# ethz-asl/okvis

Hardware: NVIDIA B200
Metric: keyframe-window optimize() iters/sec (10KF/2k-lm stereo) (higher is better)
Workload: dtype f64

## Files before the change

okvis_b200/csrc/okb_estimator.cu:

```cuda
#include <cuda_runtime.h>

#include <algorithm>
#include <cstddef>
#include <cstdio>
#include <cstdlib>
#include <cstring>
#include <string>
#include <thread>
#include <vector>

#include "okb_ctx.h"
#include "okb_hostpack.hpp"
#include "okb_graph.cuh"
#include "okb_kernels.cuh"
#include "okb_marg.cuh"

using namespace okb;

static std::string g_create_error;

#define OKB_CUDA(ctx, call)                                                                             \
  do {                                                                                                  \
    cudaError_t e_ = (call);                                                                            \
    if (e_ != cudaSuccess) {                                                                            \
      (ctx)->set_error(std::string(#call) + ": " + cudaGetErrorString(e_));                             \
      return OKB_ERR_CUDA;                                                                              \
    }                                                                                                   \
  } while (0)

static inline size_t align_up(size_t v, size_t a) { return (v + a - 1) / a * a; }

static cudaError_t create_transfer_stream(cudaStream_t* s) {
  int lo = 0, hi = 0;
  cudaDeviceGetStreamPriorityRange(&lo, &hi);
  return cudaStreamCreateWithPriority(s, cudaStreamNonBlocking, hi);
}

extern "C" int okb_ctx_create(int device_id, int max_windows, okb_ctx** out) {
  if (!out || max_windows < 1) return OKB_ERR_INVALID_ARG;
  *out = nullptr;
  int n = 0;
  cudaError_t e = cudaGetDeviceCount(&n);
  if (e != cudaSuccess || n == 0) {
    g_create_error = std::string("no CUDA device: ") + cudaGetErrorString(e);
    return OKB_ERR_NO_DEVICE;
  }
  if (device_id < 0 || device_id >= n) { g_create_error = "bad device id"; return OKB_ERR_INVALID_ARG; }
  okb_ctx* c = new okb_ctx();
  c->device = device_id;
  c->max_windows = max_windows;
  int prio_least = 0, prio_greatest = 0;
  if (cudaSetDevice(device_id) == cudaSuccess) cudaDeviceGetStreamPriorityRange(&prio_least, &prio_greatest);
  if (cudaSetDevice(device_id) != cudaSuccess || cudaStreamCreateWithPriority(&c->stream, cudaStreamNonBlocking, prio_greatest) != cudaSuccess) {
    g_create_error = "cudaSetDevice / cudaStreamCreate failed";
    delete c;
    return OKB_ERR_CUDA;
  }
  if (cudaStreamCreateWithPriority(&c->stream_imu, cudaStreamNonBlocking, prio_least) != cudaSuccess ||
      cudaEventCreateWithFlags(&c->ev_round, cudaEventDisableTiming) != cudaSuccess ||
      cudaEventCreateWithFlags(&c->ev_imu, cudaEventDisableTiming) != cudaSuccess ||
      create_transfer_stream(&c->stream_xfer) != cudaSuccess ||
      cudaEventCreateWithFlags(&c->ev_join, cudaEventDisableTiming) != cudaSuccess) {
    g_create_error = "cudaStreamCreate / cudaEventCreate failed";
    delete c;
    return OKB_ERR_CUDA;
  }
  for (int k = 0; k < okb_ctx::kDoneRing; ++k) cudaEventCreateWithFlags(&c->done_ring[k], cudaEventDisableTiming);
  cudaDeviceProp prop;
  cudaGetDeviceProperties(&prop, device_id);
  c->sm_count = prop.multiProcessorCount;
  c->smem_optin = (int)prop.sharedMemPerBlockOptin;
  c->smem_per_sm = (int)prop.sharedMemPerMultiprocessor;
  c->wins.resize(max_windows);
  c->host.assign(max_windows, WinDev());
  std::memset(c->host.data(), 0, sizeof(WinDev) * max_windows);
  c->chunk_cap = std::max(1, std::min(kMaxChunks, (2 * c->sm_count) / max_windows));
  if (cudaMalloc(&c->d_wins, sizeof(WinDev) * max_windows) != cudaSuccess ||
      cudaMalloc(&c->d_states, sizeof(SolverState) * max_windows) != cudaSuccess ||
      cudaMallocHost(&c->h_states, sizeof(SolverState) * max_windows) != cudaSuccess) {
    g_create_error = "cudaMalloc failed";
    delete c;
    return OKB_ERR_CUDA;
  }
  cudaMemset(c->d_states, 0, sizeof(SolverState) * max_windows);
  cudaFuncSetAttribute(k_schur, cudaFuncAttributeMaxDynamicSharedMemorySize, c->smem_optin);
  cudaFuncSetAttribute(k_imu, cudaFuncAttributeMaxDynamicSharedMemorySize, (int)smemI_bytes());
  cudaFuncSetAttribute(k_imu, cudaFuncAttributePreferredSharedMemoryCarveout, cudaSharedmemCarveoutMaxShared);
  cudaFuncSetAttribute(k_solve<S_THREADS>, cudaFuncAttributeMaxDynamicSharedMemorySize, c->smem_optin);
  cudaFuncSetAttribute(k_solve<S_THREADS>, cudaFuncAttributePreferredSharedMemoryCarveout, cudaSharedmemCarveoutMaxShared);
  cudaFuncSetAttribute(k_solve<512>, cudaFuncAttributeMaxDynamicSharedMemorySize, c->smem_optin);
  cudaFuncSetAttribute(k_solve<512>, cudaFuncAttributePreferredSharedMemoryCarveout, cudaSharedmemCarveoutMaxShared);
  cudaFuncSetAttribute(k_schur, cudaFuncAttributePreferredSharedMemoryCarveout, cudaSharedmemCarveoutMaxShared);
  cudaFuncSetAttribute(k_quality, cudaFuncAttributeMaxDynamicSharedMemorySize, c->smem_optin);
  *out = c;
  return OKB_OK;
}

extern "C" void okb_ctx_destroy(okb_ctx* c) {
  if (!c) return;
  cudaSetDevice(c->device);
  cudaStreamSynchronize(c->stream);
  if (c->stream_xfer) cudaStreamSynchronize(c->stream_xfer);
  for (auto& w : c->wins) {
    if (w.arena) cudaFree(w.arena);
    if (w.marg_scratch) cudaFree(w.marg_scratch);
    if (w.staging) cudaFreeHost(w.staging);
    if (w.out_staging) cudaFreeHost(w.out_staging);
    if (w.copied) cudaEventDestroy(w.copied);
    if (w.down) cudaEventDestroy(w.down);
  }
  for (int k = 0; k < okb_ctx::kDoneRing; ++k) if (c->done_ring[k]) cudaEventDestroy(c->done_ring[k]);
  if (c->ev_join) cudaEventDestroy(c->ev_join);
  if (c->stream_xfer) cudaStreamDestroy(c->stream_xfer);
  okb_frontend_release(c);
  for (int r = 0; r < kMaxShard; ++r)
    if (c->shard_peer_ipc[r] && c->shard_peer[r]) cudaIpcCloseMemHandle(c->shard_peer[r]);
  if (c->shard_local) cudaFree(c->shard_local);
  if (c->d_wins) cudaFree(c->d_wins);
  if (c->d_states) cudaFree(c->d_states);
  if (c->h_states) cudaFreeHost(c->h_states);
  if (c->hook_buf) cudaFree(c->hook_buf);
  for (auto& g : c->graphs) if (g.exec) cudaGraphExecDestroy(g.exec);
  for (auto e : c->prof_events) cudaEventDestroy(e);
  if (c->ev_round) cudaEventDestroy(c->ev_round);
  if (c->ev_imu) cudaEventDestroy(c->ev_imu);
  if (c->stream_imu) cudaStreamDestroy(c->stream_imu);
  cudaStreamDestroy(c->stream);
  delete c;
}

extern "C" const char* okb_last_error(const okb_ctx* c) { return c ? c->error.c_str() : g_create_error.c_str(); }
extern "C" int64_t okb_kernel_launches(const okb_ctx* c) { return c ? c->launches : 0; }
extern "C" void* okb_stream(const okb_ctx* c) { return c ? (void*)c->stream : nullptr; }

namespace {
struct ArenaPlan {
  size_t total = 0;
  size_t take(size_t bytes) {
    const size_t o = total;
    total = align_up(total + bytes, 256);
    return o;
  }
};

int join_transfers(okb_ctx* c) {
  if (cudaEventRecord(c->ev_join, c->stream_xfer) != cudaSuccess) return 1;
  return cudaStreamWaitEvent(c->stream, c->ev_join, 0) != cudaSuccess;
}
void mark_work(okb_ctx* c, int first, int count) {
  const int k = c->done_next;
  c->done_next = (k + 1) % okb_ctx::kDoneRing;
  cudaEventRecord(c->done_ring[k], c->stream);
  for (int i = first; i < first + count; ++i) c->wins[i].done_idx = k;
}

inline bool caps_cover(const WinCaps& a, const WinCaps& b) {
  return a.K >= b.K && a.L >= b.L && a.O >= b.O && a.S >= b.S && a.T >= b.T && a.NE >= b.NE && a.NC >= b.NC && a.PP >= b.PP && a.MN >= b.MN;
}
inline WinCaps caps_max(const WinCaps& a, const WinCaps& b) {
  return WinCaps{std::max(a.K, b.K), std::max(a.L, b.L), std::max(a.O, b.O), std::max(a.S, b.S), std::max(a.T, b.T),
                 std::max(a.NE, b.NE), std::max(a.NC, b.NC), std::max(a.PP, b.PP), std::max(a.MN, b.MN)};
}
inline size_t full_upload_bytes(const WinCaps& q) {
  return 12 * sizeof(CmdHeader) + 8 * ((size_t)7 * q.NE + 16 * (size_t)q.K + 4 * (size_t)q.L + 2 * kMaxMargBlocks + 16 * kMaxMargBlocks +
                                        (size_t)q.MN * q.MN + q.MN) +
         sizeof(okb_camera) * q.NC + sizeof(okb_observation) * (size_t)q.O + sizeof(okb_imu_term) * q.T + sizeof(okb_imu_sample) * (size_t)q.S +
         (sizeof(okb_pose_prior) + sizeof(okb_sb_prior)) * q.PP + 4096;
}

void derive_dims(WinDev& W) {
  int CP = 1;
  while (CP < W.NC) CP <<= 1;
  W.CP = CP;
  W.NS = W.K * CP; W.NG = (W.NS + 31) / 32; W.NSP = W.NG * 32;
  W.dc = 6 * W.K; W.d = W.dc + 9 * W.NSB; W.dcp = 4 * ((W.dc + 1 + 3) / 4);
  W.Lp = (W.L + 31) & ~31;
// ... 780 lines not shown
  out[0] = (double)s.shard_rounds; out[1] = 1e-3 * (double)s.shard_wait_ns; out[2] = (double)s.shard_fault; out[3] = (double)s.shard_epoch;
  return OKB_OK;
}

static void prof_begin(okb_ctx* c, int kind) {
  if (!c->profile) return;
  if (c->prof_used + 2 > c->prof_events.size()) {
    cudaEvent_t a, b;
    cudaEventCreate(&a); cudaEventCreate(&b);
    c->prof_events.push_back(a); c->prof_events.push_back(b);
  }
  c->prof_kind.push_back(kind);
  cudaEventRecord(c->prof_events[c->prof_used], c->stream);
}
static void prof_end(okb_ctx* c) {
  if (!c->profile) return;
  cudaEventRecord(c->prof_events[c->prof_used + 1], c->stream);
  c->prof_used += 2;
}
extern "C" int okb_profile_enable(okb_ctx* c, int on) {
  if (!c) return OKB_ERR_INVALID_ARG;
  cudaSetDevice(c->device);
  cudaStreamSynchronize(c->stream);
  c->profile = on != 0;
  c->prof_used = 0;
  c->prof_kind.clear();
  return OKB_OK;
}
extern "C" int okb_profile_read(okb_ctx* c, double out[6]) {
  if (!c || !out) return OKB_ERR_INVALID_ARG;
  cudaSetDevice(c->device);
  cudaStreamSynchronize(c->stream);
  for (int i = 0; i < 6; ++i) out[i] = 0.0;
  for (size_t i = 0; i < c->prof_kind.size(); ++i) {
    float ms = 0.f;
    cudaEventElapsedTime(&ms, c->prof_events[2 * i], c->prof_events[2 * i + 1]);
    out[2 * c->prof_kind[i]] += ms;
    out[2 * c->prof_kind[i] + 1] += 1.0;
  }
  c->prof_used = 0;
  c->prof_kind.clear();
  return OKB_OK;
}

static int check_range(okb_ctx* c, int first, int count) {
  if (!c || first < 0 || count < 1 || first + count > c->max_windows) return OKB_ERR_INVALID_ARG;
  for (int i = first; i < first + count; ++i)
    if (!c->wins[i].uploaded) { c->set_error("window slot not uploaded"); return OKB_ERR_INVALID_ARG; }
  return OKB_OK;
}

extern "C" int64_t okb_window_h2d_bytes(const okb_ctx* c, int win) {
  if (!c || win < 0 || win >= c->max_windows || !c->wins[win].uploaded) return 0;
  return (int64_t)(c->wins[win].h2d_bytes + sizeof(WinDev));
}

extern "C" int okb_window_reset(okb_ctx* c, int first, int count) {
  int rc = check_range(c, first, count);
  if (rc) return rc;
  cudaSetDevice(c->device);
  for (int i = first; i < first + count; ++i) {
    const WinStore& S = c->wins[i];
    const WinDev& W = c->host[i];
    if (W.K != S.K_init || W.NSB != S.NSB_init || W.L != S.L_init) { c->set_error("okb_window_reset: the window changed shape since its last full upload"); return OKB_ERR_INVALID_ARG; }
  }
  rc = commit_range(c, first, count);
  if (rc) return rc;
  cudaStream_t xs = c->stream_xfer;
  bool waited[okb_ctx::kDoneRing] = {};
  for (int i = first; i < first + count; ++i) {
    const WinStore& S = c->wins[i];
    if (S.done_idx >= 0 && !waited[S.done_idx]) {
      OKB_CUDA(c, cudaStreamWaitEvent(xs, c->done_ring[S.done_idx], 0));
      waited[S.done_idx] = true;
    }
  }
  k_reset<<<count, 128, 0, xs>>>(c->d_wins, first, 1);
  c->launches += 1;
  OKB_CUDA(c, cudaGetLastError());
  return OKB_OK;
}

struct RoundPlan {
  int max_chunks = 1, max_imu = 0, max_cx = 1, max_K = 1, acc_copies = 1, chol_smem = 1, solve_threads = S_THREADS, gxQ = 1, shard = 0, push_gx = 1;
  size_t smA = 0, smS = 0, smQ = 0;
};
static int plan_rounds(okb_ctx* c, int first, int count, RoundPlan& P) {
  P = RoundPlan();
  int chol_smem = 1;
  int acc_copies = 1;
  const size_t sm_two = ((size_t)c->smem_per_sm - 2048) / 2;
  for (int i = first; i < first + count; ++i)
    if (smemA2_bytes(c->host[i].K, c->host[i].dcp, 1) > std::min((size_t)c->smem_optin, sm_two) &&
        smemA2_bytes(c->host[i].K, c->host[i].dcp, 0) <= sm_two) acc_copies = 0;
  for (int i = first; i < first + count; ++i)
    if (smemA2_bytes(c->host[i].K, c->host[i].dcp, acc_copies) > (size_t)c->smem_optin) acc_copies = 0;
  int maxL = 1;
  for (int i = first; i < first + count; ++i) {
    const WinDev& W = c->host[i];
    P.max_chunks = std::max(P.max_chunks, W.n_chunks);
    P.max_imu = std::max(P.max_imu, W.n_imu);
    P.smA = std::max(P.smA, smemA2_bytes(W.K, W.dcp, acc_copies));
    P.max_cx = std::max(P.max_cx, (W.L + L1_THREADS - 1) / L1_THREADS);
    P.max_K = std::max(P.max_K, W.K);
    {
      const int wm = smemS_bytes(W.d, W.dc, W.K, W.marg_n, W.n_imu, 1) <= (size_t)c->smem_optin ? 1
                   : smemS_bytes(W.d, W.dc, W.K, W.marg_n, W.n_imu, 2) <= (size_t)c->smem_optin ? 2 : 0;
      if (wm == 0 || chol_smem == 0) chol_smem = 0;
      else if (wm == 2) chol_smem = 2;
    }
    P.smQ = std::max(P.smQ, (size_t)W.NS * sizeof(SlotCtx));
    maxL = std::max(maxL, W.L);
  }
  for (int i = first; i < first + count; ++i) {
    const WinDev& W = c->host[i];
    P.smS = std::max(P.smS, smemS_bytes(W.d, W.dc, W.K, W.marg_n, W.n_imu, chol_smem));
  }
  if (P.smS > (size_t)c->smem_optin) { c->set_error("window does not fit kernel S shared memory"); return OKB_ERR_CAPACITY; }
  if (const char* force = getenv("OKB_SOLVE_MODE")) {
    const int m = atoi(force);
    if ((m == 0 || m == 2) && chol_smem != 0 && !(chol_smem == 2 && m == 2)) {
      chol_smem = m;
      P.smS = 0;
      for (int i = first; i < first + count; ++i) {
        const WinDev& W = c->host[i];
        P.smS = std::max(P.smS, smemS_bytes(W.d, W.dc, W.K, W.marg_n, W.n_imu, chol_smem));
      }
      if (P.smS > (size_t)c->smem_optin) { c->set_error("window does not fit kernel S shared memory"); return OKB_ERR_CAPACITY; }
    }
  }
  P.acc_copies = acc_copies; P.chol_smem = chol_smem;
  P.solve_threads = (2 * count <= c->sm_count) ? 512 : S_THREADS;
  P.gxQ = std::max(1, std::min((maxL + 127) / 128, (4 * c->sm_count + count - 1) / count));
  P.shard = c->shard_world > 1 ? 1 : 0;
  P.push_gx = std::max(1, std::min(16, c->sm_count / std::max(1, count)));
  return OKB_OK;
}

static int launch_rounds(okb_ctx* c, int first, int count, const okb_solve_options& opt, int rounds, const RoundPlan& P) {
  for (int r = 0; r < rounds; ++r) {
    const dim3 gridA(P.max_chunks, count);
    static const bool imu_serial = getenv("OKB_IMU_SERIAL") != nullptr;
    if (P.max_imu > 0 && imu_serial) {
      k_imu<<<dim3((P.max_imu + 32 / IMU_G - 1) / (32 / IMU_G), count), 32, smemI_bytes(), c->stream>>>(c->d_wins, first);
      c->launches += 1;
    } else if (P.max_imu > 0) {
      cudaEventRecord(c->ev_round, c->stream);
      cudaStreamWaitEvent(c->stream_imu, c->ev_round, 0);
      k_imu<<<dim3((P.max_imu + 32 / IMU_G - 1) / (32 / IMU_G), count), 32, smemI_bytes(), c->stream_imu>>>(c->d_wins, first);
      cudaEventRecord(c->ev_imu, c->stream_imu);
      c->launches += 1;
    }
    prof_begin(c, 0);
    k_linearize<<<dim3(P.max_cx, P.max_K, count), L1_THREADS, 0, c->stream>>>(c->d_wins, first);
    k_lmblock<<<dim3(P.max_cx, count), 128, 0, c->stream>>>(c->d_wins, first);
    k_schur<<<gridA, A2_THREADS, P.smA, c->stream>>>(c->d_wins, first, P.acc_copies, opt.max_iterations);
    if (P.shard) {
      k_shard_push<<<dim3(P.push_gx, count), 256, 0, c->stream>>>(c->d_wins, first);
      c->launches += 1;
    } else if (P.max_chunks > 1) { k_reduce_partials<<<dim3(8, count), 256, 0, c->stream>>>(c->d_wins, first); c->launches += 1; }
    prof_end(c);
    c->launches += 3;
    if (P.max_imu > 0 && !imu_serial) cudaStreamWaitEvent(c->stream, c->ev_imu, 0);
    prof_begin(c, 1);
    if (P.solve_threads == 512) k_solve<512><<<count, 512, P.smS, c->stream>>>(c->d_wins, first, opt, P.chol_smem);
    else k_solve<S_THREADS><<<count, S_THREADS, P.smS, c->stream>>>(c->d_wins, first, opt, P.chol_smem);
    prof_end(c);
    c->launches += 1;
  }
  OKB_CUDA(c, cudaGetLastError());
  return OKB_OK;
}

static int launch_quality(okb_ctx* c, int first, int count, const RoundPlan& P) {
  prof_begin(c, 2);
  k_quality<<<dim3(P.gxQ, count), 128, P.smQ, c->stream>>>(c->d_wins, first);
  prof_end(c);
  c->launches += 1;
  OKB_CUDA(c, cudaGetLastError());
  return OKB_OK;
}

static int run_rounds(okb_ctx* c, int first, int count, const okb_solve_options& opt, int rounds, bool with_quality) {
  RoundPlan P;
  int rc = plan_rounds(c, first, count, P);
  if (rc) return rc;
  static const bool no_graph = getenv("OKB_NO_GRAPH") != nullptr;
  if (c->profile || no_graph || c->shard_world > 1) {
    rc = launch_rounds(c, first, count, opt, rounds, P);
    if (!rc && with_quality) rc = launch_quality(c, first, count, P);
    return rc;
  }
  okb_ctx::GraphEntry key;
  std::memset(&key, 0, sizeof key);
  key.first = first; key.count = count; key.rounds = rounds; key.with_quality = with_quality ? 1 : 0;
  key.opt_iter = opt.max_iterations; key.opt_min = opt.min_iterations; key.opt_cauchy = opt.use_cauchy_loss; key.opt_time = opt.time_limit_s;
  static_assert(sizeof(RoundPlan) <= sizeof(key.plan), "plan blob");
  std::memcpy(key.plan, &P, sizeof P);
  for (auto& e : c->graphs)
    if (e.exec && !std::memcmp(&e, &key, offsetof(okb_ctx::GraphEntry, exec))) {
      e.stamp = ++c->graph_clock;
      OKB_CUDA(c, cudaGraphLaunch(e.exec, c->stream));
      c->launches += e.launches;
      return OKB_OK;
    }
  const int64_t l0 = c->launches;
  cudaGraph_t graph = nullptr;
  OKB_CUDA(c, cudaStreamBeginCapture(c->stream, cudaStreamCaptureModeThreadLocal));
  rc = launch_rounds(c, first, count, opt, rounds, P);
  if (!rc && with_quality) rc = launch_quality(c, first, count, P);
  const cudaError_t ce = cudaStreamEndCapture(c->stream, &graph);
  if (rc) { if (graph) cudaGraphDestroy(graph); return rc; }
  OKB_CUDA(c, ce);
  key.launches = c->launches - l0;
  c->launches = l0;
  OKB_CUDA(c, cudaGraphInstantiate(&key.exec, graph, 0));
  cudaGraphDestroy(graph);
  okb_ctx::GraphEntry* slot = nullptr;
  for (auto& e : c->graphs) if (!e.exec) { slot = &e; break; }
  if (!slot && c->graphs.size() < 16) { c->graphs.emplace_back(); slot = &c->graphs.back(); }
  if (!slot) {
    slot = &c->graphs[0];
    for (auto& e : c->graphs) if (e.stamp < slot->stamp) slot = &e;
    cudaGraphExecDestroy(slot->exec);
  }
  key.stamp = ++c->graph_clock;
  *slot = key;
  OKB_CUDA(c, cudaGraphLaunch(slot->exec, c->stream));
  c->launches += slot->launches;
  return OKB_OK;
}

extern "C" int okb_optimize_async(okb_ctx* c, int first, int count, const okb_solve_options* opt) {
  int rc = check_range(c, first, count);
  if (rc) return rc;
  if (!opt || opt->max_iterations < 0) return OKB_ERR_INVALID_ARG;
  cudaSetDevice(c->device);
  rc = commit_range(c, first, count);
  if (rc) return rc;
  for (int i = first; i < first + count; ++i) {
    WinDev& W = c->host[i];
    int chunks = (2 * c->sm_count + count - 1) / count;
    chunks = std::max(1, std::min(chunks, c->chunk_cap));
    chunks = std::min(chunks, std::max(1, W.L / (2 * A2_TILE)));
    W.lm_per_chunk = (((W.L + chunks - 1) / chunks) + A2_TILE - 1) / A2_TILE * A2_TILE;
    W.n_chunks = (W.L + W.lm_per_chunk - 1) / W.lm_per_chunk;
    W.use_cauchy = opt->use_cauchy_loss ? 1 : 0;
  }
  if (join_transfers(c)) { c->set_error("stream ordering failed"); return OKB_ERR_CUDA; }
  OKB_CUDA(c, cudaMemcpyAsync(c->d_wins + first, &c->host[first], sizeof(WinDev) * count, cudaMemcpyHostToDevice, c->stream));
  k_reset<<<count, 128, 0, c->stream>>>(c->d_wins, first, 0);
  c->launches += 1;
  for (int i = first; i < first + count; ++i) c->wins[i].opt = *opt;
  rc = run_rounds(c, first, count, *opt, opt->max_iterations + 1, true);
  if (rc) return rc;
  OKB_CUDA(c, cudaMemcpyAsync(c->h_states + first, c->d_states + first, sizeof(SolverState) * count, cudaMemcpyDeviceToHost, c->stream));
  mark_work(c, first, count);
  return rc;
}
// ... 418 lines not shown
```

okvis_b200/csrc/okb_kernels_lm.cuh:

```cuda
#pragma once
#include "okb_estimator.cuh"

namespace okb {

constexpr int L1_THREADS = 128;
constexpr int A2_THREADS = 192;
constexpr int A2_TILE = 32;
constexpr int kPartH = 32;

struct SlotCtx {
  SlotXf xf;
  CamIntr cam;
  int frame;
  int valid;
};
static_assert(sizeof(SlotCtx) % 8 == 0, "SlotCtx is copied as doubles");

__device__ inline void build_slot_ctx(const WinDev& W, int tid, int nthr) {
  for (int s = tid; s < W.NS; s += nthr) {
    const SlotInfo si = W.slots[s];
    SlotCtx sc;
    sc.valid = si.valid; sc.frame = s / W.CP;
    if (si.valid) { make_slot_xf(W.pose_c + 7 * si.pose_idx, W.ext + 7 * si.ext_idx, sc.xf); cam_load(W.cams[si.cam_idx], sc.cam); }
    else { for (int k = 0; k < 9; ++k) sc.xf.R[k] = 0; for (int k = 0; k < 3; ++k) sc.xf.t[k] = 0; cam_load(W.cams[0], sc.cam); }
    W.slot_ctx[s] = sc;
  }
}

__global__ void __launch_bounds__(L1_THREADS) k_linearize(const WinDev* __restrict__ wins, int win_first) {
  const WinDev& W = wins[win_first + blockIdx.z];
  const SolverState* st = W.st;
  if (st->done) return;
  const int f = blockIdx.y;
  const int cx = blockIdx.x;
  if (f >= W.K || cx * L1_THREADS >= W.L) return;
  const int tid = threadIdx.x;
  const int L = W.L, CP = W.CP;

  __shared__ SlotCtx slots[32];
  __shared__ double sred[kPartH][L1_THREADS + 1];
  __shared__ double s_tw[3];

  if (f != 0) {
    bool any = false;
#pragma unroll
    for (int t = 0; t < L1_THREADS / 32; ++t) {
      const int tile = cx * (L1_THREADS / 32) + t;
      if (tile * 32 < L) {
        const uint32_t tr = W.tile_range[tile];
        any = any || ((int)(tr & 0xffu) <= f && f <= (int)(tr >> 8));
      }
    }
    if (!any) {
      if (tid < 29) W.partH[((size_t)cx * W.K + f) * kPartH + tid] = 0.0;
      return;
    }
  }
  const int mode = st->mode, cur = st->cur;
  const bool cauchy = W.use_cauchy != 0;
  const int l = cx * L1_THREADS + tid;
  const int lc = min(l, L - 1);
  const uint32_t vmask = W.lm_vis[lc];
  const double4 x4 = *reinterpret_cast<const double4*>(W.lm + 4 * (size_t)lc);
  const size_t gi0 = (size_t)(f * CP) * L + lc;
  double w0 = W.obs_w[gi0], w1 = 0.0;
  double2 z0 = W.obs_z[gi0], z1 = make_double2(0, 0);
  if (CP > 1) { w1 = W.obs_w[gi0 + L]; z1 = W.obs_z[gi0 + L]; }
  double sg[3] = {0, 0, 0}, sE[3] = {1, 1, 1}, sgn[3] = {0, 0, 0};
  if (mode == MODE_STEP) {
    const double* g = W.lm_g[cur] + 3 * (size_t)lc;
    const double* E = W.lm_E[cur] + 3 * (size_t)lc;
    const double* gn = W.lm_gn + 3 * (size_t)lc;
#pragma unroll
    for (int c = 0; c < 3; ++c) { sg[c] = g[c]; sE[c] = E[c]; sgn[c] = gn[c]; }
  }
  {
    const double* src = reinterpret_cast<const double*>(W.slot_ctx + f * CP);
    double* dst = reinterpret_cast<double*>(slots);
    const int n = CP * (int)(sizeof(SlotCtx) / sizeof(double));
    for (int i = tid; i < n; i += L1_THREADS) dst[i] = src[i];
  }
  if (tid < 3) s_tw[tid] = W.pose_c[7 * f + tid];
#pragma unroll
  for (int i = 0; i < 29; ++i) sred[i][tid] = 0.0;
  __syncthreads();

  if (l < L) {
    const bool vis = (vmask >> f) & 1u;
    if (vis || f == 0) {
      double X[4] = {x4.x, x4.y, x4.z, x4.w};
      if (mode == MODE_STEP) {
        const double a = st->a, b = st->b;
        double dn = 0;
#pragma unroll
        for (int c = 0; c < 3; ++c) {
          const double dlt = a * sg[c] / sE[c] + b * sgn[c];
          X[c] += dlt;
          dn += dlt * dlt;
        }
        if (f == 0) sred[28][tid] = dn;
      }
      if (f == 0) *reinterpret_cast<double4*>(W.lm_c + 4 * (size_t)l) = make_double4(X[0], X[1], X[2], X[3]);
      if (vis) {
        double M0 = 0, M1 = 0, M2 = 0, M3 = 0, M4 = 0, M5 = 0, m0 = 0, m1 = 0, m2 = 0, cost = 0, lprod = 1.0;
        auto add_obs = [&](const SlotCtx& sc, double wobs, double2 z) {
          if (wobs > 0.0 && sc.valid) {
            double r[2], A[6];
            reproj_slot<true>(sc.xf, sc.cam, X, z.x, z.y, wobs, r, A);
            const double sq = r[0] * r[0] + r[1] * r[1];
            double rho1 = 1.0;
            if (cauchy) {
              rho1 = 1.0 / (1.0 + sq);
              lprod *= 1.0 + sq;
              if (lprod > 1e250) { cost += 0.5 * log(lprod); lprod = 1.0; }
            } else cost += 0.5 * sq;
            M0 += rho1 * (A[0] * A[0] + A[3] * A[3]);
            M1 += rho1 * (A[0] * A[1] + A[3] * A[4]);
            M2 += rho1 * (A[0] * A[2] + A[3] * A[5]);
            M3 += rho1 * (A[1] * A[1] + A[4] * A[4]);
            M4 += rho1 * (A[1] * A[2] + A[4] * A[5]);
            M5 += rho1 * (A[2] * A[2] + A[5] * A[5]);
            m0 += rho1 * (A[0] * r[0] + A[3] * r[1]);
            m1 += rho1 * (A[1] * r[0] + A[4] * r[1]);
            m2 += rho1 * (A[2] * r[0] + A[5] * r[1]);
          }
        };
        add_obs(slots[0], w0, z0);
        if (CP > 1) add_obs(slots[1], w1, z1);
        for (int c = 2; c < CP; ++c) {
          const size_t gi = gi0 + (size_t)c * L;
          add_obs(slots[c], W.obs_w[gi], W.obs_z[gi]);
        }
        if (cauchy) cost += 0.5 * log(lprod);
        double* Mo = W.lm_M + lm_M_index(l, f, W.K);
        Mo[0] = M0; Mo[32] = M1; Mo[64] = M2; Mo[96] = M3; Mo[128] = M4; Mo[160] = M5;
        double* mo = W.lm_mf + lm_mf_index(l, f, W.K);
        mo[0] = m0; mo[32] = m1; mo[64] = m2;
        const double w = X[3];
        const double p0 = X[0] - s_tw[0] * w, p1 = X[1] - s_tw[1] * w, p2 = X[2] - s_tw[2] * w;
        const double Q00 = M1 * p2 - M2 * p1, Q01 = -M0 * p2 + M2 * p0, Q02 = M0 * p1 - M1 * p0;
        const double Q10 = M3 * p2 - M4 * p1, Q11 = -M1 * p2 + M4 * p0, Q12 = M1 * p1 - M3 * p0;
        const double Q20 = M4 * p2 - M5 * p1, Q21 = -M2 * p2 + M5 * p0, Q22 = M2 * p1 - M4 * p0;
        const double w2 = w * w;
        sred[0][tid] = w2 * M0; sred[1][tid] = w2 * M1; sred[2][tid] = w2 * M2; sred[3][tid] = w2 * M3; sred[4][tid] = w2 * M4; sred[5][tid] = w2 * M5;
        sred[6][tid] = -w * Q00; sred[7][tid] = -w * Q01; sred[8][tid] = -w * Q02;
        sred[9][tid] = -w * Q10; sred[10][tid] = -w * Q11; sred[11][tid] = -w * Q12;
        sred[12][tid] = -w * Q20; sred[13][tid] = -w * Q21; sred[14][tid] = -w * Q22;
        sred[15][tid] = p2 * Q10 - p1 * Q20; sred[16][tid] = p2 * Q11 - p1 * Q21; sred[17][tid] = p2 * Q12 - p1 * Q22;
        sred[18][tid] = -p2 * Q01 + p0 * Q21; sred[19][tid] = -p2 * Q02 + p0 * Q22;
        sred[20][tid] = p1 * Q02 - p0 * Q12;
        sred[21][tid] = w * m0; sred[22][tid] = w * m1; sred[23][tid] = w * m2;
        sred[24][tid] = p1 * m2 - p2 * m1; sred[25][tid] = p2 * m0 - p0 * m2; sred[26][tid] = p0 * m1 - p1 * m0;
        sred[27][tid] = cost;
      }
    }
  }
  __syncthreads();
  {
    const int e = tid >> 2, q = tid & 3;
    double s = 0.0;
    if (e < 29) {
      const double* row = &sred[e][q * 32];
#pragma unroll 8
      for (int i = 0; i < 32; ++i) s += row[(i + 4 * q) & 31];
    }
    s += __shfl_xor_sync(0xffffffffu, s, 1);
    s += __shfl_xor_sync(0xffffffffu, s, 2);
    if (e < 29 && q == 0) W.partH[((size_t)cx * W.K + f) * kPartH + e] = s;
  }
}

__global__ void __launch_bounds__(128) k_lmblock(const WinDev* __restrict__ wins, int win_first) {
  const WinDev& W = wins[win_first + blockIdx.y];
  SolverState* st = W.st;
  if (st->done) return;
  const int l = blockIdx.x * blockDim.x + threadIdx.x;
  const int L = W.L, K = W.K;
  if (l >= L) return;
  const int mode = st->mode, cur = st->cur;
  const double mu = (mode == MODE_STEP) ? fmax(kMinMu, 2.0 * st->mu / kMuIncrease) : st->mu;
  double H[6] = {0, 0, 0, 0, 0, 0}, gl[3] = {0, 0, 0};
  uint32_t vis = W.lm_vis[l];
  for (int f = 0; f < K; ++f) {
    if ((vis >> f) & 1u) {
      const double* Mo = W.lm_M + lm_M_index(l, f, K);
      const double* mo = W.lm_mf + lm_mf_index(l, f, K);
#pragma unroll
      for (int i = 0; i < 6; ++i) H[i] += Mo[32 * i];
      gl[0] -= mo[0]; gl[1] -= mo[32]; gl[2] -= mo[64];
    }
  }
  double sc3[3], E[3];
  const double hd[3] = {H[0], H[3], H[5]};
  if (mode == MODE_INIT) {
#pragma unroll
    for (int c = 0; c < 3; ++c) { sc3[c] = 1.0 / (1.0 + sqrt(hd[c])); W.lm_scale[3 * (size_t)l + c] = sc3[c]; }
  } else {
#pragma unroll
    for (int c = 0; c < 3; ++c) sc3[c] = W.lm_scale[3 * (size_t)l + c];
  }
#pragma unroll
  for (int c = 0; c < 3; ++c) {
    const double s2 = sc3[c] * sc3[c];
    E[c] = fmin(fmax(s2 * hd[c], kMinDiag), kMaxDiag) / s2;
  }
  const double R[6] = {H[0] + mu * E[0], H[1], H[2], H[3] + mu * E[1], H[4], H[5] + mu * E[2]};
  double Lc[6], Li[6];
  if (chol3(R, Lc)) linv3(Lc, Li);
  else {
#pragma unroll
    for (int i = 0; i < 6; ++i) Li[i] = 0.0;
    st->numeric_fail = 1;
  }
  double* Ro = W.lm_Rinv + 6 * (size_t)l;
  Ro[0] = Li[0] * Li[0] + Li[1] * Li[1] + Li[3] * Li[3];
  Ro[1] = Li[1] * Li[2] + Li[3] * Li[4];
  Ro[2] = Li[3] * Li[5];
  Ro[3] = Li[2] * Li[2] + Li[4] * Li[4];
  Ro[4] = Li[4] * Li[5];
  Ro[5] = Li[5] * Li[5];
  double* gs = W.lm_g[cur ^ 1] + 3 * (size_t)l;
  double* Es = W.lm_E[cur ^ 1] + 3 * (size_t)l;
#pragma unroll
  for (int c = 0; c < 3; ++c) { gs[c] = gl[c]; Es[c] = E[c]; }
  double* Lo = W.lm_Li + 9 * (size_t)l;
#pragma unroll
  for (int i = 0; i < 6; ++i) Lo[i] = Li[i];
  Lo[6] = Li[0] * gl[0];
  Lo[7] = Li[1] * gl[0] + Li[2] * gl[1];
  Lo[8] = Li[3] * gl[0] + Li[4] * gl[1] + Li[5] * gl[2];
}

constexpr int kLiStride = 9;

__host__ __device__ inline int schur_ldy(int dcp) { return dcp + 2; }

__host__ __device__ inline size_t schur_acc_doubles(int K) { return (size_t)(6 * K + 1) * (6 * K + 2) / 2; }
__host__ __device__ inline size_t smemA2_bytes(int K, int dcp, int acc_copies) {
  size_t b = 16;
  b += ((size_t)3 * A2_TILE * schur_ldy(dcp) + 8) * sizeof(double);
  b += (size_t)2 * K * 6 * A2_TILE * sizeof(double);
  b += (size_t)2 * A2_TILE * kLiStride * sizeof(double);
  b += (size_t)2 * A2_TILE * 4 * sizeof(double);
  b += (size_t)K * 4 * sizeof(double);
  b += (size_t)acc_copies * schur_acc_doubles(K) * sizeof(double);
  return b;
}

__device__ __forceinline__ uint32_t smem_u32(const void* p) { return (uint32_t)__cvta_generic_to_shared(p); }
__device__ __forceinline__ void mbar_init(uint64_t* bar, uint32_t count) {
  asm volatile("mbarrier.init.shared::cta.b64 [%0], %1;" ::"r"(smem_u32(bar)), "r"(count) : "memory");
}
__device__ __forceinline__ void mbar_arrive_expect_tx(uint64_t* bar, uint32_t bytes) {
  asm volatile("mbarrier.arrive.expect_tx.shared::cta.b64 _, [%0], %1;" ::"r"(smem_u32(bar)), "r"(bytes) : "memory");
}
__device__ __forceinline__ void bulk_g2s(void* dst, const void* src, uint32_t bytes, uint64_t* bar) {
  asm volatile("cp.async.bulk.shared::cluster.global.mbarrier::complete_tx::bytes [%0], [%1], %2, [%3];" ::"r"(smem_u32(dst)), "l"(src),
               "r"(bytes), "r"(smem_u32(bar))
               : "memory");
}
__device__ __forceinline__ void mbar_wait(uint64_t* bar, uint32_t parity) {
  uint32_t ok;
  do {
    asm volatile("{\n\t.reg .pred p;\n\tmbarrier.try_wait.parity.shared::cta.b64 p, [%1], %2;\n\tselp.u32 %0, 1, 0, p;\n\t}"
                 : "=r"(ok)
                 : "r"(smem_u32(bar)), "r"(parity)
                 : "memory");
  } while (!ok);
}
__device__ __forceinline__ void fence_proxy_async() { asm volatile("fence.proxy.async.shared::cta;" ::: "memory"); }

__global__ void __launch_bounds__(A2_THREADS, 2) k_schur(const WinDev* __restrict__ wins, int win_first, int acc_copies, int max_iterations) {
  const WinDev& W = wins[win_first + blockIdx.y];
  SolverState* st = W.st;
// ... 380 lines not shown
```

Baseline: 195,900.

## Fuse landmark block solve into linearize kernel with per-landmark frame loop

The per-(chunk, frame) linearize grid and the separate k_lmblock kernel are merged into one kernel where each thread loops over the keyframes in its tile range, accumulating the landmark H and gradient in registers. This removes one launch per round and avoids re-reading lm_M and lm_mf from global memory. The 128x29 shared reduction is replaced with a warp transpose-reduce over shuffles, and the slot contexts move into dynamic shared memory. The trade-off is less parallelism, since frames are now processed serially per block, plus a __syncthreads per frame.

Result: faster. 227,800, median of 6 (+16.3%).

```diff
diff --git a/okvis_b200/csrc/okb_estimator.cu b/okvis_b200/csrc/okb_estimator.cu
--- a/okvis_b200/csrc/okb_estimator.cu
+++ b/okvis_b200/csrc/okb_estimator.cu
@@ -92,6 +92,11 @@
   cudaFuncSetAttribute(k_solve<512>, cudaFuncAttributePreferredSharedMemoryCarveout, cudaSharedmemCarveoutMaxShared);
   cudaFuncSetAttribute(k_schur, cudaFuncAttributePreferredSharedMemoryCarveout, cudaSharedmemCarveoutMaxShared);
   cudaFuncSetAttribute(k_quality, cudaFuncAttributeMaxDynamicSharedMemorySize, c->smem_optin);
+  {
+    cudaFuncAttributes fa;
+    if (cudaFuncGetAttributes(&fa, k_linearize) == cudaSuccess)
+      cudaFuncSetAttribute(k_linearize, cudaFuncAttributeMaxDynamicSharedMemorySize, c->smem_optin - (int)fa.sharedSizeBytes);
+  }
   *out = c;
   return OKB_OK;
 }
@@ -1038,8 +1043,8 @@
 }
 
 struct RoundPlan {
-  int max_chunks = 1, max_imu = 0, max_cx = 1, max_K = 1, acc_copies = 1, chol_smem = 1, solve_threads = S_THREADS, gxQ = 1, shard = 0, push_gx = 1;
-  size_t smA = 0, smS = 0, smQ = 0;
+  int max_chunks = 1, max_imu = 0, max_cx = 1, acc_copies = 1, chol_smem = 1, solve_threads = S_THREADS, gxQ = 1, shard = 0, push_gx = 1;
+  size_t smA = 0, smS = 0, smSlots = 0;
 };
 static int plan_rounds(okb_ctx* c, int first, int count, RoundPlan& P) {
   P = RoundPlan();
@@ -1058,14 +1063,13 @@
     P.max_imu = std::max(P.max_imu, W.n_imu);
     P.smA = std::max(P.smA, smemA2_bytes(W.K, W.dcp, acc_copies));
     P.max_cx = std::max(P.max_cx, (W.L + L1_THREADS - 1) / L1_THREADS);
-    P.max_K = std::max(P.max_K, W.K);
     {
       const int wm = smemS_bytes(W.d, W.dc, W.K, W.marg_n, W.n_imu, 1) <= (size_t)c->smem_optin ? 1
                    : smemS_bytes(W.d, W.dc, W.K, W.marg_n, W.n_imu, 2) <= (size_t)c->smem_optin ? 2 : 0;
       if (wm == 0 || chol_smem == 0) chol_smem = 0;
       else if (wm == 2) chol_smem = 2;
     }
-    P.smQ = std::max(P.smQ, (size_t)W.NS * sizeof(SlotCtx));
+    P.smSlots = std::max(P.smSlots, (size_t)W.NS * sizeof(SlotCtx));
     maxL = std::max(maxL, W.L);
   }
   for (int i = first; i < first + count; ++i) {
@@ -1108,15 +1112,14 @@
       c->launches += 1;
     }
     prof_begin(c, 0);
-    k_linearize<<<dim3(P.max_cx, P.max_K, count), L1_THREADS, 0, c->stream>>>(c->d_wins, first);
-    k_lmblock<<<dim3(P.max_cx, count), 128, 0, c->stream>>>(c->d_wins, first);
+    k_linearize<<<dim3(P.max_cx, count), L1_THREADS, P.smSlots, c->stream>>>(c->d_wins, first);
     k_schur<<<gridA, A2_THREADS, P.smA, c->stream>>>(c->d_wins, first, P.acc_copies, opt.max_iterations);
     if (P.shard) {
       k_shard_push<<<dim3(P.push_gx, count), 256, 0, c->stream>>>(c->d_wins, first);
       c->launches += 1;
     } else if (P.max_chunks > 1) { k_reduce_partials<<<dim3(8, count), 256, 0, c->stream>>>(c->d_wins, first); c->launches += 1; }
     prof_end(c);
-    c->launches += 3;
+    c->launches += 2;
     if (P.max_imu > 0 && !imu_serial) cudaStreamWaitEvent(c->stream, c->ev_imu, 0);
     prof_begin(c, 1);
     if (P.solve_threads == 512) k_solve<512><<<count, 512, P.smS, c->stream>>>(c->d_wins, first, opt, P.chol_smem);
@@ -1130,7 +1133,7 @@
 
 static int launch_quality(okb_ctx* c, int first, int count, const RoundPlan& P) {
   prof_begin(c, 2);
-  k_quality<<<dim3(P.gxQ, count), 128, P.smQ, c->stream>>>(c->d_wins, first);
+  k_quality<<<dim3(P.gxQ, count), 128, P.smSlots, c->stream>>>(c->d_wins, first);
   prof_end(c);
   c->launches += 1;
   OKB_CUDA(c, cudaGetLastError());
diff --git a/okvis_b200/csrc/okb_kernels_lm.cuh b/okvis_b200/csrc/okb_kernels_lm.cuh
--- a/okvis_b200/csrc/okb_kernels_lm.cuh
+++ b/okvis_b200/csrc/okb_kernels_lm.cuh
@@ -4,6 +4,7 @@
 namespace okb {
 
 constexpr int L1_THREADS = 128;
+constexpr int L1_MIN_CTAS = 4;
 constexpr int A2_THREADS = 192;
 constexpr int A2_TILE = 32;
 constexpr int kPartH = 32;
@@ -27,84 +28,104 @@
   }
 }
 
-__global__ void __launch_bounds__(L1_THREADS) k_linearize(const WinDev* __restrict__ wins, int win_first) {
-  const WinDev& W = wins[win_first + blockIdx.z];
-  const SolverState* st = W.st;
+template <class V>
+__device__ __forceinline__ double warp_transpose_reduce32(const V& v, int lane) {
+  double r[16];
+  const bool up16 = lane & 16;
+#pragma unroll
+  for (int i = 0; i < 16; ++i) {
+    const double lo = v(i), hi = v(i + 16);
+    r[i] = (up16 ? hi : lo) + __shfl_xor_sync(0xffffffffu, up16 ? lo : hi, 16);
+  }
+#pragma unroll
+  for (int h = 8; h >= 1; h >>= 1) {
+    const bool up = lane & h;
+#pragma unroll
+    for (int i = 0; i < h; ++i) {
+      const double lo = r[i], hi = r[i + h];
+      r[i] = (up ? hi : lo) + __shfl_xor_sync(0xffffffffu, up ? lo : hi, h);
+    }
+  }
+  return r[0];
+}
+
+__global__ void __launch_bounds__(L1_THREADS, L1_MIN_CTAS) k_linearize(const WinDev* __restrict__ wins, int win_first) {
+  const WinDev& W = wins[win_first + blockIdx.y];
+  SolverState* st = W.st;
   if (st->done) return;
-  const int f = blockIdx.y;
+  const int L = W.L, K = W.K, CP = W.CP;
   const int cx = blockIdx.x;
-  if (f >= W.K || cx * L1_THREADS >= W.L) return;
-  const int tid = threadIdx.x;
-  const int L = W.L, CP = W.CP;
-
-  __shared__ SlotCtx slots[32];
-  __shared__ double sred[kPartH][L1_THREADS + 1];
-  __shared__ double s_tw[3];
-
-  if (f != 0) {
-    bool any = false;
-#pragma unroll
-    for (int t = 0; t < L1_THREADS / 32; ++t) {
-      const int tile = cx * (L1_THREADS / 32) + t;
-      if (tile * 32 < L) {
-        const uint32_t tr = W.tile_range[tile];
-        any = any || ((int)(tr & 0xffu) <= f && f <= (int)(tr >> 8));
-      }
-    }
-    if (!any) {
-      if (tid < 29) W.partH[((size_t)cx * W.K + f) * kPartH + tid] = 0.0;
-      return;
-    }
-  }
+  if (cx * L1_THREADS >= L) return;
+  const int tid = threadIdx.x, warp = tid >> 5, lane = tid & 31;
+  const int l = cx * L1_THREADS + tid;
+  const bool live = l < L;
+
+  __shared__ double s_red[2][L1_THREADS / 32][32];
+  __shared__ double s_dn[L1_THREADS / 32];
+  extern __shared__ __align__(16) unsigned char smem_raw[];
+  SlotCtx* s_sl = reinterpret_cast<SlotCtx*>(smem_raw);
+
+  int fa = K, fb = -1, Fa = K, Fb = -1;
+#pragma unroll
+  for (int t = 0; t < L1_THREADS / 32; ++t) {
+    const int tile = cx * (L1_THREADS / 32) + t;
+    if (tile * 32 < L) {
+      const uint32_t tr = W.tile_range[tile];
+      const int a = (int)(tr & 0xffu), b = (int)(tr >> 8);
+      if (a <= b) {
+        Fa = min(Fa, a); Fb = max(Fb, b);
+        if (t == warp) { fa = a; fb = b; }
+      }
+    }
+  }
+
   const int mode = st->mode, cur = st->cur;
   const bool cauchy = W.use_cauchy != 0;
-  const int l = cx * L1_THREADS + tid;
-  const int lc = min(l, L - 1);
-  const uint32_t vmask = W.lm_vis[lc];
-  const double4 x4 = *reinterpret_cast<const double4*>(W.lm + 4 * (size_t)lc);
-  const size_t gi0 = (size_t)(f * CP) * L + lc;
-  double w0 = W.obs_w[gi0], w1 = 0.0;
-  double2 z0 = W.obs_z[gi0], z1 = make_double2(0, 0);
-  if (CP > 1) { w1 = W.obs_w[gi0 + L]; z1 = W.obs_z[gi0 + L]; }
-  double sg[3] = {0, 0, 0}, sE[3] = {1, 1, 1}, sgn[3] = {0, 0, 0};
-  if (mode == MODE_STEP) {
-    const double* g = W.lm_g[cur] + 3 * (size_t)lc;
-    const double* E = W.lm_E[cur] + 3 * (size_t)lc;
-    const double* gn = W.lm_gn + 3 * (size_t)lc;
-#pragma unroll
-    for (int c = 0; c < 3; ++c) { sg[c] = g[c]; sE[c] = E[c]; sgn[c] = gn[c]; }
-  }
-  {
-    const double* src = reinterpret_cast<const double*>(W.slot_ctx + f * CP);
-    double* dst = reinterpret_cast<double*>(slots);
-    const int n = CP * (int)(sizeof(SlotCtx) / sizeof(double));
-    for (int i = tid; i < n; i += L1_THREADS) dst[i] = src[i];
-  }
-  if (tid < 3) s_tw[tid] = W.pose_c[7 * f + tid];
-#pragma unroll
-  for (int i = 0; i < 29; ++i) sred[i][tid] = 0.0;
+  const uint32_t vmask = live ? W.lm_vis[l] : 0u;
+  double X[4] = {0.0, 0.0, 0.0, 1.0};
+  double dn = 0.0;
+  if (live) {
+    const double4 x4 = *reinterpret_cast<const double4*>(W.lm + 4 * (size_t)l);
+    X[0] = x4.x; X[1] = x4.y; X[2] = x4.z; X[3] = x4.w;
+    if (mode == MODE_STEP) {
+      const double a = st->a, b = st->b;
+      const double* g = W.lm_g[cur] + 3 * (size_t)l;
+      const double* E = W.lm_E[cur] + 3 * (size_t)l;
+      const double* gn = W.lm_gn + 3 * (size_t)l;
+#pragma unroll
+      for (int c = 0; c < 3; ++c) {
+        const double dlt = a * g[c] / E[c] + b * gn[c];
+        X[c] += dlt;
+        dn += dlt * dlt;
+      }
+    }
+    *reinterpret_cast<double4*>(W.lm_c + 4 * (size_t)l) = make_double4(X[0], X[1], X[2], X[3]);
+  }
+#pragma unroll
+  for (int o = 16; o > 0; o >>= 1) dn += __shfl_xor_sync(0xffffffffu, dn, o);
+  if (lane == 0) s_dn[warp] = dn;
+  if (Fa <= Fb) {
+    constexpr int nd = (int)(sizeof(SlotCtx) / sizeof(double));
+    const double* src = reinterpret_cast<const double*>(W.slot_ctx);
+    double* dst = reinterpret_cast<double*>(s_sl);
+    for (int i = Fa * CP * nd + tid; i < (Fb + 1) * CP * nd; i += L1_THREADS) dst[i] = src[i];
+  }
   __syncthreads();
 
-  if (l < L) {
+  double H0 = 0, H1 = 0, H2 = 0, H3 = 0, H4 = 0, H5 = 0, gl0 = 0, gl1 = 0, gl2 = 0;
+  for (int f = Fa; f <= Fb; ++f) {
     const bool vis = (vmask >> f) & 1u;
-    if (vis || f == 0) {
-      double X[4] = {x4.x, x4.y, x4.z, x4.w};
-      if (mode == MODE_STEP) {
-        const double a = st->a, b = st->b;
-        double dn = 0;
-#pragma unroll
-        for (int c = 0; c < 3; ++c) {
-          const double dlt = a * sg[c] / sE[c] + b * sgn[c];
-          X[c] += dlt;
-          dn += dlt * dlt;
-        }
-        if (f == 0) sred[28][tid] = dn;
-      }
-      if (f == 0) *reinterpret_cast<double4*>(W.lm_c + 4 * (size_t)l) = make_double4(X[0], X[1], X[2], X[3]);
+    double* sr = s_red[f & 1][warp];
+    if (f >= fa && f <= fb && __any_sync(0xffffffffu, vis)) {
+      double M0 = 0, M1 = 0, M2 = 0, M3 = 0, M4 = 0, M5 = 0, m0 = 0, m1 = 0, m2 = 0, cost = 0;
       if (vis) {
-        double M0 = 0, M1 = 0, M2 = 0, M3 = 0, M4 = 0, M5 = 0, m0 = 0, m1 = 0, m2 = 0, cost = 0, lprod = 1.0;
-        auto add_obs = [&](const SlotCtx& sc, double wobs, double2 z) {
+        double lprod = 1.0;
+        for (int c = 0; c < CP; ++c) {
+          const size_t gi = (size_t)(f * CP + c) * L + l;
+          const double wobs = W.obs_w[gi];
+          const SlotCtx& sc = s_sl[f * CP + c];
           if (wobs > 0.0 && sc.valid) {
+            const double2 z = W.obs_z[gi];
             double r[2], A[6];
             reproj_slot<true>(sc.xf, sc.cam, X, z.x, z.y, wobs, r, A);
             const double sq = r[0] * r[0] + r[1] * r[1];
@@ -124,72 +145,68 @@
             m1 += rho1 * (A[1] * r[0] + A[4] * r[1]);
             m2 += rho1 * (A[2] * r[0] + A[5] * r[1]);
           }
-        };
-        add_obs(slots[0], w0, z0);
-        if (CP > 1) add_obs(slots[1], w1, z1);
-        for (int c = 2; c < CP; ++c) {
-          const size_t gi = gi0 + (size_t)c * L;
-          add_obs(slots[c], W.obs_w[gi], W.obs_z[gi]);
         }
         if (cauchy) cost += 0.5 * log(lprod);
-        double* Mo = W.lm_M + lm_M_index(l, f, W.K);
+        double* Mo = W.lm_M + lm_M_index(l, f, K);
         Mo[0] = M0; Mo[32] = M1; Mo[64] = M2; Mo[96] = M3; Mo[128] = M4; Mo[160] = M5;
-        double* mo = W.lm_mf + lm_mf_index(l, f, W.K);
+        double* mo = W.lm_mf + lm_mf_index(l, f, K);
         mo[0] = m0; mo[32] = m1; mo[64] = m2;
-        const double w = X[3];
-        const double p0 = X[0] - s_tw[0] * w, p1 = X[1] - s_tw[1] * w, p2 = X[2] - s_tw[2] * w;
-        const double Q00 = M1 * p2 - M2 * p1, Q01 = -M0 * p2 + M2 * p0, Q02 = M0 * p1 - M1 * p0;
-        const double Q10 = M3 * p2 - M4 * p1, Q11 = -M1 * p2 + M4 * p0, Q12 = M1 * p1 - M3 * p0;
-        const double Q20 = M4 * p2 - M5 * p1, Q21 = -M2 * p2 + M5 * p0, Q22 = M2 * p1 - M4 * p0;
-        const double w2 = w * w;
-        sred[0][tid] = w2 * M0; sred[1][tid] = w2 * M1; sred[2][tid] = w2 * M2; sred[3][tid] = w2 * M3; sred[4][tid] = w2 * M4; sred[5][tid] = w2 * M5;
-        sred[6][tid] = -w * Q00; sred[7][tid] = -w * Q01; sred[8][tid] = -w * Q02;
-        sred[9][tid] = -w * Q10; sred[10][tid] = -w * Q11; sred[11][tid] = -w * Q12;
-        sred[12][tid] = -w * Q20; sred[13][tid] = -w * Q21; sred[14][tid] = -w * Q22;
-        sred[15][tid] = p2 * Q10 - p1 * Q20; sred[16][tid] = p2 * Q11 - p1 * Q21; sred[17][tid] = p2 * Q12 - p1 * Q22;
-        sred[18][tid] = -p2 * Q01 + p0 * Q21; sred[19][tid] = -p2 * Q02 + p0 * Q22;
-        sred[20][tid] = p1 * Q02 - p0 * Q12;
-        sred[21][tid] = w * m0; sred[22][tid] = w * m1; sred[23][tid] = w * m2;
-        sred[24][tid] = p1 * m2 - p2 * m1; sred[25][tid] = p2 * m0 - p0 * m2; sred[26][tid] = p0 * m1 - p1 * m0;
-        sred[27][tid] = cost;
-      }
+        H0 += M0; H1 += M1; H2 += M2; H3 += M3; H4 += M4; H5 += M5;
+        gl0 -= m0; gl1 -= m1; gl2 -= m2;
+      }
+      const double w = vis ? X[3] : 0.0;
+      const double* tw = W.pose_c + 7 * f;
+      const double p0 = vis ? X[0] - tw[0] * w : 0.0, p1 = vis ? X[1] - tw[1] * w : 0.0, p2 = vis ? X[2] - tw[2] * w : 0.0;
+      const double Q00 = M1 * p2 - M2 * p1, Q01 = -M0 * p2 + M2 * p0, Q02 = M0 * p1 - M1 * p0;
+      const double Q10 = M3 * p2 - M4 * p1, Q11 = -M1 * p2 + M4 * p0, Q12 = M1 * p1 - M3 * p0;
+      const double Q20 = M4 * p2 - M5 * p1, Q21 = -M2 * p2 + M5 * p0, Q22 = M2 * p1 - M4 * p0;
+      const double w2 = w * w;
+      auto val = [&](int e) -> double {
+        switch (e) {
+          case 0: return w2 * M0;  case 1: return w2 * M1;  case 2: return w2 * M2;
+          case 3: return w2 * M3;  case 4: return w2 * M4;  case 5: return w2 * M5;
+          case 6: return -w * Q00; case 7: return -w * Q01; case 8: return -w * Q02;
+          case 9: return -w * Q10; case 10: return -w * Q11; case 11: return -w * Q12;
+          case 12: return -w * Q20; case 13: return -w * Q21; case 14: return -w * Q22;
+          case 15: return p2 * Q10 - p1 * Q20; case 16: return p2 * Q11 - p1 * Q21; case 17: return p2 * Q12 - p1 * Q22;
+          case 18: return -p2 * Q01 + p0 * Q21; case 19: return -p2 * Q02 + p0 * Q22;
+          case 20: return p1 * Q02 - p0 * Q12;
+          case 21: return w * m0;  case 22: return w * m1;  case 23: return w * m2;
+          case 24: return p1 * m2 - p2 * m1; case 25: return p2 * m0 - p0 * m2; case 26: return p0 * m1 - p1 * m0;
+          case 27: return cost;
+          default: return 0.0;
+        }
+      };
+      sr[lane] = warp_transpose_reduce32(val, lane);
+    } else {
+      sr[lane] = 0.0;
+    }
+    __syncthreads();
+    if (warp == (f & (L1_THREADS / 32 - 1)) && lane < 28) {
+      double s = 0.0;
+#pragma unroll
+      for (int q = 0; q < L1_THREADS / 32; ++q) s += s_red[f & 1][q][lane];
+      W.partH[((size_t)cx * K + f) * kPartH + lane] = s;
     }
   }
   __syncthreads();
-  {
-    const int e = tid >> 2, q = tid & 3;
-    double s = 0.0;
-    if (e < 29) {
-      const double* row = &sred[e][q * 32];
-#pragma unroll 8
-      for (int i = 0; i < 32; ++i) s += row[(i + 4 * q) & 31];
-    }
-    s += __shfl_xor_sync(0xffffffffu, s, 1);
-    s += __shfl_xor_sync(0xffffffffu, s, 2);
-    if (e < 29 && q == 0) W.partH[((size_t)cx * W.K + f) * kPartH + e] = s;
-  }
-}
-
-__global__ void __launch_bounds__(128) k_lmblock(const WinDev* __restrict__ wins, int win_first) {
-  const WinDev& W = wins[win_first + blockIdx.y];
-  SolverState* st = W.st;
-  if (st->done) return;
-  const int l = blockIdx.x * blockDim.x + threadIdx.x;
-  const int L = W.L, K = W.K;
-  if (l >= L) return;
-  const int mode = st->mode, cur = st->cur;
+  for (int i = tid; i < 29 * K; i += L1_THREADS) {
+    const int f = i / 29, e = i % 29;
+    double* rec = W.partH + ((size_t)cx * K + f) * kPartH;
+    if (e == 28) {
+      double s = 0.0;
+      if (f == 0)
+#pragma unroll
+        for (int q = 0; q < L1_THREADS / 32; ++q) s += s_dn[q];
+      rec[28] = s;
+    } else if (f < Fa || f > Fb) {
+      rec[e] = 0.0;
+    }
+  }
+  if (!live) return;
+
   const double mu = (mode == MODE_STEP) ? fmax(kMinMu, 2.0 * st->mu / kMuIncrease) : st->mu;
-  double H[6] = {0, 0, 0, 0, 0, 0}, gl[3] = {0, 0, 0};
-  uint32_t vis = W.lm_vis[l];
-  for (int f = 0; f < K; ++f) {
-    if ((vis >> f) & 1u) {
-      const double* Mo = W.lm_M + lm_M_index(l, f, K);
-      const double* mo = W.lm_mf + lm_mf_index(l, f, K);
-#pragma unroll
-      for (int i = 0; i < 6; ++i) H[i] += Mo[32 * i];
-      gl[0] -= mo[0]; gl[1] -= mo[32]; gl[2] -= mo[64];
-    }
-  }
+  const double H[6] = {H0, H1, H2, H3, H4, H5}, gl[3] = {gl0, gl1, gl2};
   double sc3[3], E[3];
   const double hd[3] = {H[0], H[3], H[5]};
   if (mode == MODE_INIT) {
```
